# lxd99/TPNet

Hardware: NVIDIA B200
Metric: temporal edges/sec (update+pairwise encode) (higher is better)
Workload: dtype f32

## Files before the change

include/tpnet_b200.h:

```cpp
#ifndef TPNET_B200_H_
#define TPNET_B200_H_

#include <stddef.h>
#include <stdint.h>

#ifdef __cplusplus
extern "C" {
#endif

#define TPN_ABI_VERSION 13

#define TPN_MAX_LAYERS 4

enum {
    TPN_OK = 0,
    TPN_ERR_INVALID_ARGUMENT = -1,
    TPN_ERR_WORKSPACE_TOO_SMALL = -2,
    TPN_ERR_LOG_FULL = -3,
    TPN_ERR_CUDA = -4,
    TPN_ERR_UNSUPPORTED = -5,
    TPN_ERR_INDEX = -6
};

typedef struct tpn_state {
    float*   data;
    int64_t  num_nodes;
    int32_t  num_layer;
    int32_t  dim;
    int64_t  row_stride;
    int64_t  node_stride;
    int32_t* stamps;
    double*  decay_log;
    int64_t  log_capacity;
    int64_t  epoch;
    double   cum_floor;
    int32_t* err_flag;
    int32_t  giant_chunk;
    int32_t  reserved0;
} tpn_state_t;

int tpn_version(void);
const char* tpn_error_string(int code);
const char* tpn_last_cuda_error(void);
int tpn_device_info(int* sm_count, int* cc_major, int* cc_minor);

size_t tpn_update_workspace_bytes(const tpn_state_t* st, int64_t batch);

int tpn_update(tpn_state_t* st,
               const int64_t* src_dev, const int64_t* dst_dev, const double* t_dev, int64_t batch,
               double t_last, float neg_lambda, const float* decay,
               void* ws_dev, size_t ws_bytes, int32_t* err_flag_dev, void* stream);

#define TPN_UPDATE_WHOLE 0
#define TPN_UPDATE_PREPARE 1
#define TPN_UPDATE_APPLY 2
int tpn_update_phase(tpn_state_t* st,
                     const int64_t* src_dev, const int64_t* dst_dev, const double* t_dev, int64_t batch,
                     double t_last, float neg_lambda, const float* decay,
                     void* ws_dev, size_t ws_bytes, int32_t* err_flag_dev, void* stream, int phase);

#define TPN_DEBUG_PER_LAYER_WALK 1
#define TPN_DEBUG_SERIAL_WALK 2
#define TPN_DEBUG_SNAPSHOT_P0 4
#define TPN_DEBUG_HEAD_FFMA 8
#define TPN_DEBUG_LEGACY_FRONT 16
#define TPN_DEBUG_NO_STREAM 32
#define TPN_DEBUG_STREAM_ALL 64
int tpn_set_debug_flags(int flags);


int tpn_update_messages(tpn_state_t* st,
                        const int64_t* tgt_dev, const int64_t* src_dev, const double* t_dev, int64_t num_messages,
                        const int32_t* num_messages_dev, int64_t num_local_rows,
                        double t_last, float neg_lambda, const float* decay,
                        void* ws_dev, size_t ws_bytes, int32_t* err_flag_dev, void* stream);

int tpn_gather_blocks(const tpn_state_t* st, const int64_t* ids_dev, int64_t n, float* out_dev, void* stream);

int tpn_pairwise(const tpn_state_t* st, const int64_t* a_ids_dev, const int64_t* b_ids_dev, int64_t n,
                 const int32_t* n_dev, int apply_log_scale, float* out_dev, void* stream);

int tpn_pairwise_neighbors(const tpn_state_t* st, const int64_t* nbr_dev, const int64_t* src_dev,
                           const int64_t* dst_dev, int64_t m, int num_neighbors, int apply_log_scale,
                           float* out_dev, void* stream);

int tpn_head_forward(const float* x_dev, int64_t n, const int32_t* n_dev, int features, int hidden, const float* w1_dev,
                     const float* b1_dev, const float* w2_dev, const float* b2_dev, float* y_dev, void* stream);

int tpn_gather(const tpn_state_t* st, const int64_t* ids_dev, int64_t n, float* out_dev, void* stream);

int tpn_materialize(tpn_state_t* st, void* stream);
int tpn_reset_epoch(tpn_state_t* st, void* stream);

int tpn_clear_walk_layers(tpn_state_t* st, void* stream);

typedef struct tpn_stager tpn_stager_t;
#define TPN_STAGE_RAW 0
#define TPN_STAGE_ID_WRAP 1
#define TPN_STAGE_ID 2
int tpn_stager_create(tpn_stager_t** out, size_t slot_bytes, int slots);
void tpn_stager_destroy(tpn_stager_t* sg);
int tpn_stage(tpn_stager_t* sg, const void* const* host, const int64_t* elems, const int* kinds, int count,
              int64_t num_nodes, void** dev_out, void* stream);

int tpn_sampler_recent(const int64_t* offsets_dev, const int64_t* nbr_dev, const int64_t* eid_dev,
                       const double* times_dev, int64_t num_nodes, const int64_t* q_nodes_dev,
                       const double* q_times_dev, int64_t n, int num_neighbors, int64_t* out_nbr_dev,
                       int64_t* out_eid_dev, double* out_times_dev, void* stream);

#define TPN_STREAM_ERR_INDEX 1
#define TPN_STREAM_ERR_ORDER 2
#define TPN_STREAM_ERR_PAST 4
typedef struct tpn_stream_sampler {
    int64_t   num_nodes;
    int32_t   capacity;
    int32_t   reserved0;
    int64_t   max_batch;
    int64_t*  all_nbr;
    int64_t*  all_eid;
    double*   all_t;
    int64_t*  old_nbr;
    int64_t*  old_eid;
    double*   old_t;
    int32_t*  all_cnt;
    int32_t*  old_cnt;
    double*   newest;
    uint32_t* pend_node;
    int64_t*  pend_nbr;
    int64_t*  pend_eid;
    double*   pend_t;
    int32_t*  pend_count;
    double*   last_time;
    int32_t*  err_flag;
} tpn_stream_sampler_t;

size_t tpn_stream_sampler_workspace_bytes(int64_t batch);
int tpn_stream_sampler_reset(const tpn_stream_sampler_t* s, void* stream);
int tpn_stream_sampler_push(const tpn_stream_sampler_t* s, const int64_t* src_dev, const int64_t* dst_dev,
                            const int64_t* eid_dev, const double* t_dev, int64_t batch, void* ws_dev, size_t ws_bytes,
                            void* stream);
int tpn_stream_sampler_query(const tpn_stream_sampler_t* s, const int64_t* q_nodes_dev, const double* q_times_dev,
                             int64_t n, int num_neighbors, int64_t* out_nbr_dev, int64_t* out_eid_dev,
                             double* out_times_dev, void* stream);

typedef struct tpn_planner tpn_planner_t;
int tpn_planner_create(tpn_planner_t** out, int64_t global_nodes, int world, int rank);
void tpn_planner_destroy(tpn_planner_t* p);
int tpn_plan(tpn_planner_t* p, const int64_t* first, const int64_t* second, int64_t count, int64_t n_local,
             int64_t* keep, int64_t* first_rows, int64_t* second_rows, int64_t* n_keep,
             int64_t* send_rows, int64_t* n_send, int64_t* send_counts, int64_t* recv_counts);

#define TPN_SHARD_CTR_NEED 0
#define TPN_SHARD_CTR_PREV 1
#define TPN_SHARD_CTR_ERROR 2
#define TPN_SHARD_COUNTERS 8
typedef struct tpn_shard {
    int32_t  world, rank;
    int64_t  global_nodes;
    int64_t  num_local_rows;
    int64_t  ext_rows;
    const float* const* peer_data;
    const int32_t* const* peer_stamps;
    uint32_t* const* peer_flags;
    int32_t* mark;
    int32_t* counters;
    int64_t* need_nodes;
    uint32_t* barrier_seq;
} tpn_shard_t;

size_t tpn_route_workspace_bytes(int64_t items);
int tpn_route_update(const tpn_shard_t* sh, const int64_t* src_dev, const int64_t* dst_dev, const double* t_dev,
                     int64_t batch, int64_t* tgt_rows_out, int64_t* src_rows_out, double* t_out,
                     int32_t* count_out_dev, void* ws_dev, size_t ws_bytes, void* stream);
int tpn_route_pairs(const tpn_shard_t* sh, const int64_t* a_dev, const int64_t* b_dev, int64_t n,
                    int64_t* a_rows_out, int64_t* b_rows_out, int64_t* keep_out, int32_t* count_out_dev,
                    void* ws_dev, size_t ws_bytes, void* stream);
int tpn_route_nodes(const tpn_shard_t* sh, const int64_t* ids_dev, int64_t n, int64_t* rows_out_dev, void* stream);
int tpn_pull_rows(const tpn_state_t* st, const tpn_shard_t* sh, void* stream);
int tpn_peer_barrier(const tpn_shard_t* sh, void* stream);
int tpn_shard_new_generation(const tpn_shard_t* sh, void* stream);
int tpn_peer_alloc(void** out, size_t bytes);
int tpn_peer_free(void* p);
int tpn_ipc_export(const void* p, unsigned char* handle64);
int tpn_ipc_open(const unsigned char* handle64, void** out);
int tpn_ipc_close(void* p);

#ifdef __cplusplus
}
#endif
#endif
```

tpnet_b200/csrc/tpn_pairwise.cu:

```cuda
#include "tpn_pairwise.cuh"

namespace tpn {
namespace {

thread_local int g_dev_slot = 0;


template <int LAYERS, int G, bool LAZY>
__global__ void __launch_bounds__(kPairThreads)
pairwise_kernel(StateView st, const long long* __restrict__ a_ids, const long long* __restrict__ b_ids,
                long long n, int apply_log_scale, float* __restrict__ out, int ds4, const int* __restrict__ n_dev) {
    if (n_dev != nullptr) {
        if (*n_dev > n && st.err != nullptr) *st.err = 4;
        n = min(n, (long long)max(*n_dev, 0));
    }
    constexpr int H = LAYERS + 1;
    constexpr int R = 2 * H;
    constexpr int F = R * R;
    constexpr int NU = R * (R + 1) / 2;
    constexpr int PPW = 32 / G;
    __shared__ __align__(16) float tile[kPairThreads / 32][PPW * F];
    __shared__ unsigned short tab[kPairThreads / 32][NU];

    const int warp = threadIdx.x >> 5;
    const int lane = threadIdx.x & 31;
    const int sub = lane / G;
    const int gl = lane % G;
    const long long pair0 = ((long long)blockIdx.x * (kPairThreads / 32) + warp) * PPW;
    if (pair0 >= n) return;
    const long long pair = pair0 + sub;
    const long long pc = pair < n ? pair : n - 1;

    long long ida = a_ids[pc], idb = b_ids[pc];
    fill_entry_table<R>(tab[warp], lane);
    ida = resolve_id(st, ida, true);
    idb = resolve_id(st, idb, true);
    const int rs4 = (int)(st.row_stride >> 2);
    const float4* pa = reinterpret_cast<const float4*>(st.data + ida * st.node_stride);
    const float4* pb = reinterpret_cast<const float4*>(st.data + idb * st.node_stride);

    float fac[R];
    if (LAZY) {
#pragma unroll
        for (int l = 1; l < H; ++l) {
            const long long sa = st.stamps[ida * LAYERS + (l - 1)];
            const long long sb = st.stamps[idb * LAYERS + (l - 1)];
            fac[l] = sa >= 0 ? decay_factor(st, l - 1, sa) : 1.0f;
            fac[H + l] = sb >= 0 ? decay_factor(st, l - 1, sb) : 1.0f;
        }
    }

    float2 acc[NU];
#pragma unroll
    for (int i = 0; i < NU; ++i) acc[i] = make_float2(0.f, 0.f);

    for (int c = gl; c < ds4; c += G) {
        float4 x[R];
#pragma unroll
        for (int l = 0; l < H; ++l) {
            x[l] = pa[l * rs4 + c];
            x[H + l] = pb[l * rs4 + c];
        }
        if (LAZY) {
#pragma unroll
            for (int l = 1; l < H; ++l) {
                scale4(x[l], fac[l]);
                scale4(x[H + l], fac[H + l]);
            }
        }
        gram_step<R>(acc, x);
    }

    __syncwarp();
    finish_pair<R, G>(acc, gl, &tile[warp][sub * F], tab[warp], apply_log_scale);
    __syncwarp();
    const long long left = n - pair0;
    const int valid = (int)(left < PPW ? left : PPW) * F;
    float* dst = out + pair0 * F;
    const float* srcs = &tile[warp][0];
    for (int i = lane * 4; i < valid; i += 32 * 4) {
        const float4 v = *reinterpret_cast<const float4*>(srcs + i);
        __stcs(reinterpret_cast<float4*>(dst + i), v);
    }
}

template <int LAYERS, bool LAZY>
__global__ void __launch_bounds__(kPairThreads)
pairwise_tma_kernel(StateView st, const long long* __restrict__ a_ids, const long long* __restrict__ b_ids,
                    long long n, int apply_log_scale, float* __restrict__ out, int ds4, const int* __restrict__ n_dev) {
    if (n_dev != nullptr) {
        if (*n_dev > n && st.err != nullptr) *st.err = 4;
        n = min(n, (long long)max(*n_dev, 0));
    }
    constexpr int G = 8;
    constexpr int H = LAYERS + 1;
    constexpr int R = 2 * H;
    constexpr int F = R * R;
    constexpr int NU = R * (R + 1) / 2;
    constexpr int PPW = 4;
    extern __shared__ __align__(128) unsigned char smem_raw[];
    __shared__ __align__(8) uint64_t mbar[kPairThreads / 32];
    __shared__ unsigned short tab[kPairThreads / 32][NU];

    const int warp = threadIdx.x >> 5;
    const int lane = threadIdx.x & 31;
    const int sub = lane / G;
    const int gl = lane % G;
    const long long pair0 = ((long long)blockIdx.x * (kPairThreads / 32) + warp) * PPW;
    if (pair0 >= n) return;
    const long long pair = pair0 + sub;
    const long long pc = pair < n ? pair : n - 1;

    long long ida = a_ids[pc], idb = b_ids[pc];
    uint64_t* bar = &mbar[warp];
    if (lane == 0) {
        mbar_init(bar, 1);
        asm volatile("fence.mbarrier_init.release.cluster;" ::: "memory");
    }
    fill_entry_table<R>(tab[warp], lane);
    ida = resolve_id(st, ida, true);
    idb = resolve_id(st, idb, true);

    const int rs4 = (int)(st.row_stride >> 2);
    const uint32_t block_bytes = (uint32_t)(H * st.row_stride * 4);
    unsigned char* wbase = smem_raw + (size_t)warp * (2 * PPW) * block_bytes;

    long long bid[PPW];
#pragma unroll
    for (int s = 0; s < PPW; ++s) bid[s] = __shfl_sync(0xffffffffu, idb, s * G);
    int sb = sub;
#pragma unroll
    for (int s = PPW - 1; s >= 1; --s)
        if (sb == s && bid[s] == bid[s - 1]) sb = s - 1;
    __syncwarp();
    if (lane == 0) {
        uint32_t copies = PPW;
#pragma unroll
        for (int s = 0; s < PPW; ++s) copies += (s == 0 || bid[s] != bid[s - 1]) ? 1u : 0u;
        mbar_expect_tx(bar, copies * block_bytes);
    }
    __syncwarp();
    if (gl == 0) {
        bulk_g2s(wbase + (size_t)sub * block_bytes, st.data + ida * st.node_stride, block_bytes, bar);
        if (sb == sub)
            bulk_g2s(wbase + (size_t)(PPW + sub) * block_bytes, st.data + idb * st.node_stride, block_bytes, bar);
    }

    float fac[R];
    if (LAZY) {
#pragma unroll
        for (int l = 1; l < H; ++l) {
            const long long sa = st.stamps[ida * LAYERS + (l - 1)];
            const long long sb = st.stamps[idb * LAYERS + (l - 1)];
            fac[l] = sa >= 0 ? decay_factor(st, l - 1, sa) : 1.0f;
            fac[H + l] = sb >= 0 ? decay_factor(st, l - 1, sb) : 1.0f;
        }
    }
    float2 acc[NU];
#pragma unroll
    for (int i = 0; i < NU; ++i) acc[i] = make_float2(0.f, 0.f);

    const float4* pa = reinterpret_cast<const float4*>(wbase + (size_t)sub * block_bytes);
    const float4* pb = reinterpret_cast<const float4*>(wbase + (size_t)(PPW + sb) * block_bytes);
    mbar_wait(bar, 0);

    for (int c = gl; c < ds4; c += G) {
        float4 x[R];
#pragma unroll
        for (int l = 0; l < H; ++l) {
            x[l] = pa[l * rs4 + c];
            x[H + l] = pb[l * rs4 + c];
        }
        if (LAZY) {
#pragma unroll
            for (int l = 1; l < H; ++l) {
                scale4(x[l], fac[l]);
                scale4(x[H + l], fac[H + l]);
            }
        }
        gram_step<R>(acc, x);
    }

    __syncwarp();
    float* tile = reinterpret_cast<float*>(wbase);
    finish_pair<R, G>(acc, gl, tile + sub * F, tab[warp], apply_log_scale);
    __syncwarp();
    const long long left = n - pair0;
    const int valid = (int)(left < PPW ? left : PPW) * F;
    float* dst = out + pair0 * F;
    for (int i = lane * 4; i < valid; i += 32 * 4) {
        const float4 v = *reinterpret_cast<const float4*>(tile + i);
        __stcs(reinterpret_cast<float4*>(dst + i), v);
    }
}

template <int LAYERS>
bool launch_tma(const StateView& v, const long long* a, const long long* b, long long n, const int* n_dev, int scale, float* out,
                cudaStream_t s) {
    constexpr int R = 2 * (LAYERS + 1);
    const size_t block_bytes = (size_t)(LAYERS + 1) * v.row_stride * 4;
    const size_t smem = (size_t)(kPairThreads / 32) * 8 * block_bytes;
    if (smem > 110 * 1024 || 4 * R * R * sizeof(float) > 8 * block_bytes || (block_bytes & 15) != 0 ||
        (v.node_stride & 3) != 0)
        return false;
    static bool configured_tab[kMaxDevices][2];
    bool* configured = configured_tab[g_dev_slot];
    const bool lazy = v.stamps != nullptr;
    auto kernel = lazy ? pairwise_tma_kernel<LAYERS, true> : pairwise_tma_kernel<LAYERS, false>;
    if (!configured[lazy ? 1 : 0]) {
        if (cudaFuncSetAttribute(kernel, cudaFuncAttributeMaxDynamicSharedMemorySize, 110 * 1024) != cudaSuccess) {
            (void)cudaGetLastError();
            return false;
        }
        configured[lazy ? 1 : 0] = true;
    }
    const unsigned grid = (unsigned)((n + 15) / 16);
    kernel<<<grid, kPairThreads, smem, s>>>(v, a, b, n, scale, out, (int)(v.row_stride / 4), n_dev);
    return true;
}

template <int LAYERS, int G>
void launch_g(const StateView& v, const long long* a, const long long* b, long long n, const int* n_dev, int scale, float* out,
              cudaStream_t s) {
    constexpr int pairs_per_block = kPairThreads / G;
    const unsigned grid = (unsigned)((n + pairs_per_block - 1) / pairs_per_block);
    const int ds4 = (int)(v.row_stride / 4);
    if (v.stamps != nullptr)
        pairwise_kernel<LAYERS, G, true><<<grid, kPairThreads, 0, s>>>(v, a, b, n, scale, out, ds4, n_dev);
    else
        pairwise_kernel<LAYERS, G, false><<<grid, kPairThreads, 0, s>>>(v, a, b, n, scale, out, ds4, n_dev);
}

template <int LAYERS>
void launch(const StateView& v, const long long* a, const long long* b, long long n, const int* n_dev, int scale, float* out,
            cudaStream_t s) {
    if (n <= 4096) {
        launch_g<LAYERS, 32>(v, a, b, n, n_dev, scale, out, s);
    } else if (!launch_tma<LAYERS>(v, a, b, n, n_dev, scale, out, s)) {
        launch_g<LAYERS, 8>(v, a, b, n, n_dev, scale, out, s);
    }
}

}
}

extern "C" int tpn_pairwise(const tpn_state_t* st, const int64_t* a_ids_dev, const int64_t* b_ids_dev, int64_t n,
                            const int32_t* n_dev, int apply_log_scale, float* out_dev, void* stream_v) {
    using namespace tpn;
    int rc = validate_state(st);
    if (rc != TPN_OK) return rc;
    if (n < 0 || n > (int64_t)1 << 34) return TPN_ERR_INVALID_ARGUMENT;
    if (n == 0) return TPN_OK;
    if (a_ids_dev == nullptr || b_ids_dev == nullptr || out_dev == nullptr ||
        (reinterpret_cast<uintptr_t>(out_dev) & 15) != 0)
        return TPN_ERR_INVALID_ARGUMENT;
    DeviceScope scope(st->data);
    g_dev_slot = scope.slot();
    cudaStream_t stream = reinterpret_cast<cudaStream_t>(stream_v);
    const StateView v = make_view(st);
    const long long* a = reinterpret_cast<const long long*>(a_ids_dev);
    const long long* b = reinterpret_cast<const long long*>(b_ids_dev);
    const int* nd = reinterpret_cast<const int*>(n_dev);
    switch (st->num_layer) {
        case 1: launch<1>(v, a, b, n, nd, apply_log_scale, out_dev, stream); break;
        case 2: launch<2>(v, a, b, n, nd, apply_log_scale, out_dev, stream); break;
        case 3: launch<3>(v, a, b, n, nd, apply_log_scale, out_dev, stream); break;
        case 4: launch<4>(v, a, b, n, nd, apply_log_scale, out_dev, stream); break;
        default: return TPN_ERR_UNSUPPORTED;
    }
    return check_launch();
}
```

Baseline: 154.6 million.

## Add persistent chunked TMA-pipelined pairwise kernel with tensor-map bulk loads

Adds a persistent pairwise kernel in which each warp walks many 4-pair tiles. Node blocks are fetched with cp.async.bulk.tensor through cached CUtensorMaps and split into column chunks on separate mbarriers, so loads for the next tile overlap the Gram computation on the current one. The grid is sized to the resident CTA count found by an occupancy query. The kernel becomes the default for large batches, with the old TMA path still reachable through a debug flag. The cost is extra host-side tensor-map encoding and caching under a mutex, plus more complex synchronisation.

New measurement: 162.6 million (median of 6 runs). 1.05x the previous value.

```diff
diff --git a/include/tpnet_b200.h b/include/tpnet_b200.h
--- a/include/tpnet_b200.h
+++ b/include/tpnet_b200.h
@@ -66,6 +66,7 @@
 #define TPN_DEBUG_LEGACY_FRONT 16
 #define TPN_DEBUG_NO_STREAM 32
 #define TPN_DEBUG_STREAM_ALL 64
+#define TPN_DEBUG_LEGACY_PAIRWISE 128
 int tpn_set_debug_flags(int flags);
 
 
diff --git a/tpnet_b200/csrc/tpn_pairwise.cu b/tpnet_b200/csrc/tpn_pairwise.cu
--- a/tpnet_b200/csrc/tpn_pairwise.cu
+++ b/tpnet_b200/csrc/tpn_pairwise.cu
@@ -1,3 +1,9 @@
+#include <cuda.h>
+#include <cudaTypedefs.h>
+#include <string.h>
+
+#include <mutex>
+
 #include "tpn_pairwise.cuh"
 
 namespace tpn {
@@ -192,6 +198,316 @@
         const float4 v = *reinterpret_cast<const float4*>(tile + i);
         __stcs(reinterpret_cast<float4*>(dst + i), v);
     }
+}
+
+#ifndef TPN_PAIRWISE_CHUNKS
+#define TPN_PAIRWISE_CHUNKS 2
+#endif
+#ifndef TPN_PAIRWISE_CTA_WARPS
+#define TPN_PAIRWISE_CTA_WARPS 4
+#endif
+constexpr int kPipeChunks = TPN_PAIRWISE_CHUNKS;
+constexpr int kPipeWarps = TPN_PAIRWISE_CTA_WARPS;
+constexpr size_t kPipeSmemPerWarp = 110 * 1024 / 4;
+
+struct PipeChunks {
+    int col0[kPipeChunks];
+    int w[kPipeChunks];
+    int buf4[kPipeChunks];
+    int slot4[kPipeChunks];
+    int warp4;
+};
+struct PipeMaps {
+    CUtensorMap m[kPipeChunks];
+};
+
+struct PipeTile {
+    long long ida, idb;
+    int sb;
+    uint32_t nblk;
+    int node;
+};
+
+__device__ __forceinline__ void pipe_prepare(const StateView& st, long long ida, long long idb, int lane, PipeTile& t) {
+    constexpr int G = 8, PPW = 4;
+    t.ida = resolve_id(st, ida, true);
+    t.idb = resolve_id(st, idb, true);
+    long long bid[PPW];
+#pragma unroll
+    for (int s = 0; s < PPW; ++s) bid[s] = __shfl_sync(0xffffffffu, t.idb, s * G);
+    const int sub = lane / G;
+    int sb = sub;
+#pragma unroll
+    for (int s = PPW - 1; s >= 1; --s)
+        if (sb == s && bid[s] == bid[s - 1]) sb = s - 1;
+    t.sb = sb;
+    uint32_t nblk = PPW;
+#pragma unroll
+    for (int s = 0; s < PPW; ++s) nblk += (s == 0 || bid[s] != bid[s - 1]) ? 1u : 0u;
+    t.nblk = nblk;
+    const int owner = (lane & (PPW - 1)) * G;
+    const long long ia = __shfl_sync(0xffffffffu, t.ida, owner);
+    const long long ib = __shfl_sync(0xffffffffu, t.idb, owner);
+    const int osb = __shfl_sync(0xffffffffu, sb, owner);
+    t.node = lane < PPW ? (int)ia : (lane < 2 * PPW && osb == lane - PPW) ? (int)ib : -1;
+}
+
+__device__ __forceinline__ void pipe_issue(const PipeTile& t, const CUtensorMap* map, float4* buf, int slot4,
+                                           uint64_t* bar, int H, int col0, int w, int lane) {
+    if (lane == 0) mbar_expect_tx(bar, t.nblk * (uint32_t)(H * w * 16));
+    __syncwarp();
+    if (t.node >= 0)
+        asm volatile(
+            "cp.async.bulk.tensor.3d.shared::cluster.global.tile.mbarrier::complete_tx::bytes [%0], [%1, {%2, %3, %4}], [%5];"
+            ::"r"(smem_u32(buf + (size_t)lane * slot4)), "l"(reinterpret_cast<uint64_t>(map)), "r"(4 * col0), "r"(0),
+              "r"(t.node), "r"(smem_u32(bar))
+            : "memory");
+}
+
+template <int LAYERS, bool LAZY>
+__device__ __forceinline__ void pipe_factors(const StateView& st, long long ida, long long idb, float (&fac)[2 * (LAYERS + 1)]) {
+    constexpr int H = LAYERS + 1;
+    if (LAZY) {
+#pragma unroll
+        for (int l = 1; l < H; ++l) {
+            const long long sa = st.stamps[ida * LAYERS + (l - 1)];
+            const long long sb = st.stamps[idb * LAYERS + (l - 1)];
+            fac[l] = sa >= 0 ? decay_factor(st, l - 1, sa) : 1.0f;
+            fac[H + l] = sb >= 0 ? decay_factor(st, l - 1, sb) : 1.0f;
+        }
+    }
+}
+
+inline int pipe_slot4(int H, int w) { return (H * w + 7) & ~7; }
+
+template <int LAYERS, bool LAZY>
+__global__ void __launch_bounds__(kPipeWarps * 32)
+pairwise_pipe_kernel(StateView st, const long long* __restrict__ a_ids, const long long* __restrict__ b_ids,
+                     long long n, int apply_log_scale, float* __restrict__ out, int ds4, const PipeChunks ck,
+                     const __grid_constant__ PipeMaps maps, const int* __restrict__ n_dev) {
+    if (n_dev != nullptr) {
+        if (*n_dev > n && st.err != nullptr) *st.err = 4;
+        n = min(n, (long long)max(*n_dev, 0));
+    }
+    constexpr int G = 8;
+    constexpr int H = LAYERS + 1;
+    constexpr int R = 2 * H;
+    constexpr int F = R * R;
+    constexpr int NU = R * (R + 1) / 2;
+    constexpr int PPW = 4;
+    constexpr int K = kPipeChunks;
+    extern __shared__ __align__(128) unsigned char smem_raw[];
+    __shared__ __align__(8) uint64_t mbar[kPipeWarps][K];
+    __shared__ unsigned short tab[kPipeWarps][NU];
+
+    const int warp = threadIdx.x >> 5;
+    const int lane = threadIdx.x & 31;
+    const int sub = lane / G;
+    const int gl = lane % G;
+    const long long tiles = (n + PPW - 1) / PPW;
+    const long long tstride = (long long)gridDim.x * kPipeWarps;
+    long long t = (long long)blockIdx.x * kPipeWarps + warp;
+    if (t >= tiles) return;
+
+    float4* region = reinterpret_cast<float4*>(smem_raw) + (size_t)warp * ck.warp4;
+    if (lane == 0) {
+#pragma unroll
+        for (int j = 0; j < K; ++j) mbar_init(&mbar[warp][j], 1);
+        asm volatile("fence.mbarrier_init.release.cluster;" ::: "memory");
+    }
+    fill_entry_table<R>(tab[warp], lane);
+    __syncwarp();
+
+    PipeTile cur;
+    float fac[R];
+    {
+        const long long pc = min(t * PPW + sub, n - 1);
+        pipe_prepare(st, a_ids[pc], b_ids[pc], lane, cur);
+#pragma unroll
+        for (int j = 0; j < K; ++j)
+            pipe_issue(cur, &maps.m[j], region + ck.buf4[j], ck.slot4[j], &mbar[warp][j], H, ck.col0[j], ck.w[j], lane);
+        pipe_factors<LAYERS, LAZY>(st, cur.ida, cur.idb, fac);
+    }
+    for (uint32_t phase = 0;; phase ^= 1u) {
+        const long long tn = t + tstride;
+        const bool more = tn < tiles;
+        long long na = 0, nb = 0;
+        if (more) {
+            const long long pc = min(tn * PPW + sub, n - 1);
+            na = a_ids[pc];
+            nb = b_ids[pc];
+        }
+        float2 acc[NU];
+#pragma unroll
+        for (int i = 0; i < NU; ++i) acc[i] = make_float2(0.f, 0.f);
+
+        PipeTile nxt;
+        float fac_n[R];
+        int c = gl;
+#pragma unroll
+        for (int j = 0; j < K; ++j) {
+            const float4* buf = region + ck.buf4[j];
+            const float4* pa = buf + sub * ck.slot4[j];
+            const float4* pb = buf + (PPW + cur.sb) * ck.slot4[j];
+            const int w = ck.w[j], c0 = ck.col0[j];
+            mbar_wait(&mbar[warp][j], phase);
+            for (; c < c0 + w; c += G) {
+                float4 x[R];
+#pragma unroll
+                for (int l = 0; l < H; ++l) {
+                    x[l] = pa[l * w + (c - c0)];
+                    x[H + l] = pb[l * w + (c - c0)];
+                }
+                if (LAZY) {
+#pragma unroll
+                    for (int l = 1; l < H; ++l) {
+                        scale4(x[l], fac[l]);
+                        scale4(x[H + l], fac[H + l]);
+                    }
+                }
+                gram_step<R>(acc, x);
+            }
+            if (j < K - 1 && more) {
+                if (j == 0) pipe_prepare(st, na, nb, lane, nxt);
+                __syncwarp();
+                pipe_issue(nxt, &maps.m[j], region + ck.buf4[j], ck.slot4[j], &mbar[warp][j], H, c0, w, lane);
+                if (j == 0) pipe_factors<LAYERS, LAZY>(st, nxt.ida, nxt.idb, fac_n);
+            }
+        }
+
+        __syncwarp();
+        float* tile = reinterpret_cast<float*>(region + ck.buf4[K - 1]);
+        finish_pair<R, G>(acc, gl, tile + sub * F, tab[warp], apply_log_scale);
+        __syncwarp();
+        const long long pair0 = t * PPW;
+        const long long left = n - pair0;
+        const int valid = (int)(left < PPW ? left : PPW) * F;
+        float* dst = out + pair0 * F;
+        for (int i = lane * 4; i < valid; i += 32 * 4) {
+            const float4 v = *reinterpret_cast<const float4*>(tile + i);
+            __stcs(reinterpret_cast<float4*>(dst + i), v);
+        }
+        if (!more) break;
+        fence_proxy_async_smem();
+        __syncwarp();
+        pipe_issue(nxt, &maps.m[K - 1], region + ck.buf4[K - 1], ck.slot4[K - 1], &mbar[warp][K - 1], H,
+                   ck.col0[K - 1], ck.w[K - 1], lane);
+        cur = nxt;
+#pragma unroll
+        for (int i = 0; i < R; ++i) fac[i] = fac_n[i];
+        t = tn;
+    }
+}
+
+bool encode_chunk_map(CUtensorMap* map, const StateView& v, int H, int w) {
+    static const PFN_cuTensorMapEncodeTiled_v12000 encode = [] {
+        void* fn = nullptr;
+        cudaDriverEntryPointQueryResult q;
+        if (cudaGetDriverEntryPoint("cuTensorMapEncodeTiled", &fn, cudaEnableDefault, &q) != cudaSuccess ||
+            q != cudaDriverEntryPointSuccess) {
+            (void)cudaGetLastError();
+            fn = nullptr;
+        }
+        return reinterpret_cast<PFN_cuTensorMapEncodeTiled_v12000>(fn);
+    }();
+    if (encode == nullptr) return false;
+    const cuuint64_t dims[3] = {(cuuint64_t)v.row_stride, (cuuint64_t)H, (cuuint64_t)v.num_nodes};
+    const cuuint64_t strides[2] = {(cuuint64_t)v.row_stride * 4, (cuuint64_t)v.node_stride * 4};
+    const cuuint32_t box[3] = {(cuuint32_t)(4 * w), (cuuint32_t)H, 1};
+    const cuuint32_t elem[3] = {1, 1, 1};
+    return encode(map, CU_TENSOR_MAP_DATA_TYPE_FLOAT32, 3, v.data, dims, strides, box, elem, CU_TENSOR_MAP_INTERLEAVE_NONE,
+                  CU_TENSOR_MAP_SWIZZLE_NONE, CU_TENSOR_MAP_L2_PROMOTION_L2_256B,
+                  CU_TENSOR_MAP_FLOAT_OOB_FILL_NONE) == CUDA_SUCCESS;
+}
+
+size_t pipe_layout(int H, int ds4, PipeChunks& ck) {
+    int col = 0, off = 0;
+    for (int j = 0; j < kPipeChunks; ++j) {
+        const int left = ds4 - col, parts = kPipeChunks - j;
+        int w = (left + parts - 1) / parts;
+        if (j < kPipeChunks - 1) {
+            int best = w;
+            for (int x = w; x <= w + 3 && x < left - (parts - 1) + 1; ++x)
+                if (pipe_slot4(H, x) - H * x < pipe_slot4(H, best) - H * best) best = x;
+            w = best;
+        } else {
+            w = left;
+        }
+        ck.col0[j] = col;
+        ck.w[j] = w;
+        ck.slot4[j] = pipe_slot4(H, w);
+        ck.buf4[j] = off;
+        off += 8 * ck.slot4[j];
+        col += w;
+    }
+    ck.warp4 = off;
+    return (size_t)off * 16;
+}
+
+struct PipeHost {
+    bool configured = false;
+    size_t occ_smem = 0;
+    int occ_per_sm = 0;
+    const void* map_data = nullptr;
+    long long map_nodes = -1, map_rs = -1, map_ns = -1;
+    PipeChunks map_ck{};
+    PipeMaps maps;
+};
+std::mutex g_pipe_mutex;
+
+template <int LAYERS>
+bool launch_pipe(const StateView& v, const long long* a, const long long* b, long long n, const int* n_dev, int scale,
+                 float* out, cudaStream_t s) {
+    constexpr int H = LAYERS + 1;
+    constexpr int R = 2 * H;
+    const int ds4 = (int)(v.row_stride / 4);
+    if (ds4 < kPipeChunks) return false;
+    PipeChunks ck;
+    const size_t per_warp = pipe_layout(H, ds4, ck);
+    const size_t smem = (size_t)kPipeWarps * per_warp;
+    bool fits = per_warp <= kPipeSmemPerWarp && 4 * R * R * sizeof(float) <= (size_t)8 * ck.slot4[kPipeChunks - 1] * 16 &&
+                (v.node_stride & 3) == 0 && v.num_nodes <= INT32_MAX;
+    for (int j = 0; j < kPipeChunks; ++j) fits = fits && ck.w[j] >= 1 && 4 * ck.w[j] <= 256;
+    if (!fits) return false;
+    const bool lazy = v.stamps != nullptr;
+    auto kernel = lazy ? pairwise_pipe_kernel<LAYERS, true> : pairwise_pipe_kernel<LAYERS, false>;
+    static PipeHost hosts[kMaxDevices][2];
+    std::lock_guard<std::mutex> lock(g_pipe_mutex);
+    PipeHost& hs = hosts[g_dev_slot][lazy ? 1 : 0];
+    if (!hs.configured) {
+        if (cudaFuncSetAttribute(kernel, cudaFuncAttributeMaxDynamicSharedMemorySize,
+                                 (int)(kPipeWarps * kPipeSmemPerWarp)) != cudaSuccess) {
+            (void)cudaGetLastError();
+            return false;
+        }
+        hs.configured = true;
+    }
+    if (hs.occ_smem != smem) {
+        int per_sm = 0;
+        if (cudaOccupancyMaxActiveBlocksPerMultiprocessor(&per_sm, kernel, kPipeWarps * 32, smem) != cudaSuccess ||
+            per_sm < 1) {
+            (void)cudaGetLastError();
+            return false;
+        }
+        hs.occ_smem = smem;
+        hs.occ_per_sm = per_sm;
+    }
+    if (hs.map_data != v.data || hs.map_nodes != v.num_nodes || hs.map_rs != v.row_stride || hs.map_ns != v.node_stride ||
+        memcmp(&hs.map_ck, &ck, sizeof ck) != 0) {
+        hs.map_data = nullptr;
+        for (int j = 0; j < kPipeChunks; ++j)
+            if (!encode_chunk_map(&hs.maps.m[j], v, H, ck.w[j])) return false;
+        hs.map_data = v.data;
+        hs.map_nodes = v.num_nodes;
+        hs.map_rs = v.row_stride;
+        hs.map_ns = v.node_stride;
+        hs.map_ck = ck;
+    }
+    const long long ctas_needed = (n + 4 * kPipeWarps - 1) / (4 * kPipeWarps);
+    const long long resident_ctas = (long long)hs.occ_per_sm * device_sm_count();
+    const unsigned grid = (unsigned)(ctas_needed < resident_ctas ? ctas_needed : resident_ctas);
+    kernel<<<grid, kPipeWarps * 32, smem, s>>>(v, a, b, n, scale, out, ds4, ck, hs.maps, n_dev);
+    return true;
 }
 
 template <int LAYERS>
@@ -236,9 +552,12 @@
             cudaStream_t s) {
     if (n <= 4096) {
         launch_g<LAYERS, 32>(v, a, b, n, n_dev, scale, out, s);
-    } else if (!launch_tma<LAYERS>(v, a, b, n, n_dev, scale, out, s)) {
+        return;
+    }
+    if ((debug_flags() & TPN_DEBUG_LEGACY_PAIRWISE) == 0 && launch_pipe<LAYERS>(v, a, b, n, n_dev, scale, out, s))
+        return;
+    if (!launch_tma<LAYERS>(v, a, b, n, n_dev, scale, out, s))
         launch_g<LAYERS, 8>(v, a, b, n, n_dev, scale, out, s);
-    }
 }
 
 }
```
